# COMP6248-Reproducability-Challenge/selfsupervised-denoising

Measured on AMD Instinct MI355X. Metric: training patches/sec (64x64 gauss25 SSDN), higher is better.
Workload: dtype f16

## Files before the change

selfsupervised-denoising_amd/csrc/wgrad_body.h:

```cpp
#pragma once
#include "common.h"
#include <algorithm>
#include <cstdlib>
#include <cstring>
#include <mutex>
#include <utility>
#include <vector>
#include <type_traits>

template <int I, int N, class F>
static __device__ __forceinline__ void static_for(F&& f) {
    if constexpr (I < N) {
        f(std::integral_constant<int, I>{});
        static_for<I + 1, N>(f);
    }
}

#define WG_THREADS 256
#define WG_WAVES 4

typedef __attribute__((__vector_size__(4 * sizeof(__fp16)))) __fp16 fp16x4_t;
typedef __attribute__((address_space(3))) fp16x4_t lds_fp16x4;

static __device__ __forceinline__ half4 tr16(const char* lds_addr) {
// ... 697 lines not shown
#pragma unroll
        for (int u = 0; u < NPD; ++u) {
            const int f = tid + u * WGN_THREADS;
            const int q = f / NPD, cc = f - q * NPD;
            *reinterpret_cast<half8*>(dt + q * DSTR + cc * 16) = pd[u];
        }
#pragma unroll
        for (int u = 0; u < 2; ++u) {
            const int hp = tid + u * WGN_THREADS;
            if (hp < 324) *reinterpret_cast<half8*>(xt + hp * 16) = cvt_h8_to_bf8(px[u]);
        }
    };

    int it = 0;
    const int t0 = (int)bx;
    if (t0 < ntiles) { fetch(t0); stage(0); }
    __syncthreads();
    for (int tile = t0; tile < ntiles; tile += (int)gdx, ++it) {
        const int nxt = tile + (int)gdx;
        if (nxt < ntiles) fetch(nxt);
        const char* dt = smem + (it & 1) * (DB + XB);
        const char* xt = dt + DB;
#pragma unroll
        for (int j = 0; j < 4; ++j) {
            const int row = wave + 4 * j;
            const char* ab = dt + (row << 4) * DSTR + dlane0;
            half8 af[MT];
#pragma unroll
            for (int mt = 0; mt < MT; ++mt) af[mt] = cat8(tr16(ab + mt * 64), tr16(ab + 4 * DSTR + mt * 64));
            const char* bp = xt + row * (18 * 16) + boff;
            u16x8 bv;
#pragma unroll
            for (int q = 0; q < 8; ++q) bv[q] = *reinterpret_cast<const unsigned short*>(bp + q * 16);
            if (bmode != 0) {
#pragma unroll
                for (int q = 0; q < 8; ++q) bv[q] = bmode == 1 ? (unsigned short)0x3f80 : (unsigned short)0;
            }
            const half8 bfrag = __builtin_bit_cast(half8, bv);
#pragma unroll
            for (int mt = 0; mt < MT; ++mt)
                acc[mt] = __builtin_amdgcn_mfma_f32_32x32x16_bf16(__builtin_bit_cast(bf16x8, af[mt]), __builtin_bit_cast(bf16x8, bfrag), acc[mt], 0, 0, 0);
        }
        __syncthreads();
        if (nxt < ntiles) stage((it + 1) & 1);
        __syncthreads();
    }
    float* red = reinterpret_cast<float*>(smem);
#pragma unroll
    for (int mt = 0; mt < MT; ++mt)
#pragma unroll
        for (int r = 0; r < 16; ++r) red[((wave * MT + mt) * 16 + r) * 64 + lane] = acc[mt][r];
    __syncthreads();
    float* slab = a.slab + (long long)bx * 9 * a.Mpad * a.Kpad;
    for (int o = tid; o < MT * 16 * 64; o += WGN_THREADS) {
        const int ln = o & 63, r = (o >> 6) & 15, mt = o >> 10;
        float sum = 0.f;
#pragma unroll
        for (int w4 = 0; w4 < 4; ++w4) sum += red[((w4 * MT + mt) * 16 + r) * 64 + ln];
        const int n = ln & 31, m = mt * 32 + 8 * (r >> 2) + 4 * (ln >> 5) + (r & 3);
        if (m >= a.Mpad) continue;
        if (n < ncol) {
            const int t = n / a.kreal, c = n - t * a.kreal;
            slab[((long long)t * a.Mpad + m) * a.Kpad + c] = sum;
        } else if (n == ncol) {
            a.bslab[(long long)bx * a.Mpad + m] = sum;
        }
    }
}
static bool wgrad_thin_ok(const ssdn_wgrad_args* a) {
    static const bool off = ssdn_tuning_env("SSDN_NO_THIN_WGRAD") != nullptr;
    if (off || a->kreal < 1 || a->kreal > 3 || a->ntaps != 9 || a->csplit > 1 || a->mblocks > 1) return false;
    if ((a->H & 15) || (a->W & 15) || (a->M & 7) || a->Mpad > 96 || a->Kpad < a->kreal) return false;
    if (a->c0 > 0 ? (a->up0 || a->c1 > 0) : a->c1 <= 0) return false;
    const ssdn_view& v = a->c0 > 0 ? a->src0 : a->src1;
    if ((v.cs & 7) || (v.co & 7) || (a->dz.cs & 7) || (a->dz.co & 7)) return false;
    int mny = 0, mxy = 0, mnx = 0, mxx = 0;
    for (int t = 0; t < 9; ++t) {
        if (a->coff[t] != 0) return false;
        mny = a->dy[t] < mny ? a->dy[t] : mny; mxy = a->dy[t] > mxy ? a->dy[t] : mxy;
        mnx = a->dx[t] < mnx ? a->dx[t] : mnx; mxx = a->dx[t] > mxx ? a->dx[t] : mxx;
    }
    return mxy - mny == 2 && mxx - mnx == 2;
}
```

selfsupervised-denoising_amd/csrc/wgrad_mega.hip:

```cpp
#include "wgrad_body.h"

namespace { std::mutex g_wg_multi_mutex; }


struct WgMegaEntry {
    ssdn_wgrad_args a;
    WgAux x;
    int inst, gx, gy, pad;
};
struct WgMegaItem { int entry, bx, by, pad; };
#define WG_MEGA_INSTANCES(X) \
    X(0, 3, 7, 4, false, 192, 8, 3, 2) X(1, 3, 5, 4, false, 192, 8, 3, 2) X(2, 2, 5, 4, false, 192, 8, 3, 2) \
    X(3, 3, 4, 6, true, 832, 4, 2, 2) X(4, 3, 4, 4, false, 0, 0, 0, 0) X(5, 3, 5, 4, false, 0, 0, 0, 0) \
    X(6, 2, 5, 4, false, 0, 0, 0, 0) X(7, 1, 1, 4, false, 0, 0, 0, 0) X(8, 3, 1, 4, false, 0, 0, 0, 0) \
    X(10, 3, 5, 6, true, 0, 0, 0, 0) X(11, 2, 5, 6, true, 0, 0, 0, 0) \
    X(12, 3, 4, 6, true, 0, 0, 0, 0) X(13, 1, 1, 6, true, 0, 0, 0, 0) X(14, 3, 1, 6, true, 0, 0, 0, 0) \
    X(15, 3, 5, 2, false, 192, 8, 3, 2) X(16, 2, 5, 2, false, 192, 8, 3, 2)
typedef const __attribute__((address_space(4))) WgMegaEntry* WgMegaEntryC;
typedef const __attribute__((address_space(4))) WgMegaItem* WgMegaItemC;
__global__ __launch_bounds__(WG_THREADS) void k_wgrad_mega(const WgMegaEntry* __restrict__ ent, const WgMegaItem* __restrict__ items) {
    const unsigned long long t_start = __builtin_amdgcn_s_memrealtime();
    const WgMegaItemC it = (WgMegaItemC)(unsigned long long)(items + blockIdx.x);
    const WgMegaEntryC E4 = (WgMegaEntryC)(unsigned long long)(ent + it->entry);
    const unsigned bx = (unsigned)it->bx, by = (unsigned)it->by;
    const WgMegaEntry& E = *(const WgMegaEntry*)E4;
    const unsigned gx = (unsigned)E.gx;
    switch (E.inst) {
#define WG_X(id, mt, cpw, nl, both, ps, ks, rwx, rwd) case id: wgrad_body<mt, cpw, nl, both, ps, ks, rwx, rwd>(E.a, E.x, bx, by, gx); break;
        WG_MEGA_INSTANCES(WG_X)
#undef WG_X
        case 101: wgrad_thin_body<1>(E.a, bx, gx); break;
        case 102: wgrad_thin_body<2>(E.a, bx, gx); break;
        case 103: wgrad_thin_body<3>(E.a, bx, gx); break;
        default: break;
    }
    {
        unsigned long long* tr = E.x.trace;
        if (tr && threadIdx.x == 0) {
            tr[3 * blockIdx.x] = t_start;
            tr[3 * blockIdx.x + 1] = __builtin_amdgcn_s_memrealtime();
            tr[3 * blockIdx.x + 2] = (unsigned long long)it->entry | ((unsigned long long)bx << 16);
        }
    }
}

struct WgVariant { int thin, mt, cpw, nl, both, ps, ks, rwx, rwd; };
static WgVariant wgrad_variant(const ssdn_wgrad_args* a, const WgPrep& p) {
    WgVariant v = {};
    v.mt = p.MT; v.cpw = p.CPW;
    if (wgrad_thin_ok(a)) { v.thin = 1; return v; }
    const WgGeom& g = p.g;
    const WgItems& wi = p.wi;
    const int ksteps = (g.TN * g.TH * g.TW) >> 4;
    const bool st = !wi.both && !wi.sync && a->ltn == 0 && a->ltw >= 3 && g.ntiles > a->nslabs;
    const bool st8 = st && g.PSTR == 192 && ksteps == 8 && wi.rswx == 3 && wi.rswd == 2;
    const bool st16 = st && g.PSTR == 64 && ksteps == 16 && wi.rswx == 5 && wi.rswd == 4;
    const bool st4b = wi.both && !wi.sync && a->ltn == 0 && a->ltw >= 3 && g.ntiles > a->nslabs && g.PSTR == 832 && ksteps == 4 && wi.rswx == 2 && wi.rswd == 2;
    v.nl = wi.both ? 6 : 4; v.both = wi.both ? 1 : 0;
    if (st4b && v.mt == 3 && v.cpw == 4) { v.ps = 832; v.ks = 4; v.rwx = 2; v.rwd = 2; }
    else if (wi.both) {}
    else if (st8 && v.mt >= 2 && v.cpw >= 2) { v.ps = 192; v.ks = 8; v.rwx = 3; v.rwd = 2; if (wgrad_nl2(a, g, v.mt, v.cpw)) v.nl = 2; }
    else if (st16 && v.mt >= 2 && v.cpw <= 3) { v.ps = 64; v.ks = 16; v.rwx = 5; v.rwd = 4; }
    return v;
}
static int wgrad_mega_inst(const WgVariant& v) {
    if (v.thin) return v.mt >= 1 && v.mt <= 3 ? 100 + v.mt : -1;
#define WG_X(id, mt_, cpw_, nl_, both_, ps_, ks_, rwx_, rwd_) \
    if (v.mt == mt_ && v.cpw == cpw_ && v.nl == nl_ && (v.both != 0) == both_ && v.ps == ps_ && v.ks == ks_ && v.rwx == rwx_ && v.rwd == rwd_) return id;
    WG_MEGA_INSTANCES(WG_X)
#undef WG_X
    return -1;
}
static int wgrad_mega_prepare(const ssdn_wgrad_args* a, WgPrep* p) {
    int rc = wgrad_prepare(a, p);
    if (rc) return rc;
    if (wgrad_thin_ok(a)) {
        p->gx = a->nslabs; p->gy = 1;
        p->lds = 2 * ((size_t)256 * wg_stride(p->MT * 64) + 18 * 18 * 16);
        const size_t red = (size_t)4 * p->MT * 16 * 64 * 4;
        p->lds = p->lds > red ? p->lds : red;
    }
    return 0;
}
int wgrad_mega_ok(const ssdn_wgrad_args* a) {
    if (!a || a->mega <= 0) return 0;
    WgPrep p;
    if (wgrad_mega_prepare(a, &p)) return 0;
    return wgrad_mega_inst(wgrad_variant(a, p)) >= 0 ? 1 : 0;
}
extern "C" int ssdn_wgrad_variant(const ssdn_wgrad_args* a, int32_t* out9) {
    WgPrep p;
    int rc = wgrad_mega_prepare(a, &p);
    if (rc) return rc < -1 ? rc : -2;
    const WgVariant v = wgrad_variant(a, p);
    const int t[9] = {v.thin, v.mt, v.cpw, v.nl, v.both, v.ps, v.ks, v.rwx, v.rwd};
    for (int i = 0; i < 9; ++i) out9[i] = t[i];
    return wgrad_mega_inst(v);
}

namespace {
struct WgMegaCache {
    std::vector<char> key;
    char* dev;
    int device;
};
std::vector<WgMegaCache> g_wg_mega_cache;
}

int launch_wgrad_mega(const ssdn_wgrad_args* const* ops, int n, hipStream_t s) {
    if (n < 1 || n > WGRAD_MEGA_MAX) return ssdn_set_error("wgrad: bad mega run length %d", n);
    const int W = ops[0]->mega;
    if (W < 1 || W > 4096) return ssdn_set_error("wgrad: bad mega grid %d", W);
    std::vector<WgMegaEntry> ent((size_t)n);
    memset(ent.data(), 0, sizeof(WgMegaEntry) * (size_t)n);
    struct It { double cost; int e, bx, by; };
    std::vector<It> its;
    size_t lds = 0;
    double flops = 0, bytes = 0;
    for (int i = 0; i < n; ++i) {
        if (ops[i]->mega != W) return ssdn_set_error("wgrad: the ops of one merged launch disagree on its grid (%d vs %d)", ops[i]->mega, W);
        WgPrep p;
        int rc = wgrad_mega_prepare(ops[i], &p);
        if (rc) return rc;
        WgMegaEntry& e = ent[i];
        memcpy(&e.a, ops[i], sizeof(ssdn_wgrad_args));
        e.x = p.x;
        e.inst = wgrad_mega_inst(wgrad_variant(ops[i], p));
        if (e.inst < 0) return ssdn_set_error("wgrad: op %d of a merged run has no k_wgrad_mega instance (MT=%d CPW=%d both=%d)", i, p.MT, p.CPW, p.wi.both);
        e.gx = p.gx; e.gy = p.gy;
        lds = p.lds > lds ? p.lds : lds;
        const double px = (double)ops[i]->N * ops[i]->H * ops[i]->W;
        const int mb = ops[i]->mblocks > 1 ? ops[i]->mblocks : 1;
        const bool thin = e.inst >= 100;
        flops += thin ? 2.0 * px * ops[i]->M * ops[i]->kreal * ops[i]->ntaps : wgrad_flops(ops[i]);
        bytes += px * 2.0 * (ops[i]->M * mb + (thin ? ops[i]->kreal : ops[i]->Ktot));
        const double c = ops[i]->cost > 0.f ? (double)ops[i]->cost : 1.0;
        for (int by = 0; by < p.gy; ++by)
            for (int bx = 0; bx < p.gx; ++bx) {
                if (mb > 1 && (((bx >> 3) / mb) * 8 + (bx & 7)) >= ops[i]->nslabs) continue;
                its.push_back({c, i, bx, by});
            }
    }
    std::stable_sort(its.begin(), its.end(), [](const It& a, const It& b) { return a.cost > b.cost; });
    std::vector<WgMegaItem> items;
    for (const It& t : its) items.push_back({t.e, t.bx, t.by, 0});
    std::vector<int> starts(1, (int)items.size());
    const size_t b0 = sizeof(WgMegaEntry) * ent.size(), b1 = sizeof(WgMegaItem) * items.size(), b2 = sizeof(int) * starts.size();
    const size_t off_items = (b0 + 255) & ~(size_t)255, off_starts = (off_items + b1 + 255) & ~(size_t)255;
    std::vector<char> key(off_starts + b2, 0);
    memcpy(key.data(), ent.data(), b0);
    memcpy(key.data() + off_items, items.data(), b1);
    memcpy(key.data() + off_starts, starts.data(), b2);
    int dev = 0;
    SSDN_CHECK_HIP(hipGetDevice(&dev));
    char* dtab = nullptr;
    {
        std::lock_guard<std::mutex> lock(g_wg_multi_mutex);
        for (const WgMegaCache& c : g_wg_mega_cache)
            if (c.device == dev && c.key.size() == key.size() && !memcmp(c.key.data(), key.data(), key.size())) { dtab = c.dev; break; }
        if (!dtab) {
            if (g_wg_mega_cache.size() >= 64) {
                SSDN_CHECK_HIP(hipDeviceSynchronize());
                SSDN_CHECK_HIP(hipFree(g_wg_mega_cache.front().dev));
// ... 22 lines not shown
```

selfsupervised-denoising_amd/csrc/wgrad_mfma.hip:

```cpp
#include "wgrad_body.h"

template <int MT, int CPW, int NL, bool BOTH, int PS, int KS, int RWX, int RWD>
__global__ __launch_bounds__(WG_THREADS) void k_wgrad(ssdn_wgrad_args a, WgAux x) {
    wgrad_body<MT, CPW, NL, BOTH, PS, KS, RWX, RWD>(a, x, blockIdx.x, blockIdx.y, gridDim.x);
}

struct WgMultiEntry {
    ssdn_wgrad_args a;
    WgAux x;
    int first, gx, gy, inst;
};
#define WG_MULTI_INSTANCES(X) \
    X(0, 2, 1, 4, false) X(1, 2, 2, 4, false) X(2, 2, 3, 4, false) X(3, 2, 5, 4, false) \
    X(4, 3, 1, 4, false) X(5, 3, 2, 4, false) X(6, 3, 3, 4, false) X(7, 3, 4, 4, false) X(8, 3, 5, 4, false) \
    X(9, 3, 1, 6, true) X(10, 2, 1, 6, true) X(11, 3, 2, 6, true) X(12, 3, 4, 6, true) X(13, 2, 3, 6, true) \
    X(16, 2, 5, 6, true) X(17, 3, 5, 6, true) X(18, 3, 3, 6, true) X(19, 2, 2, 6, true)
__global__ __launch_bounds__(WG_THREADS) void k_wgrad_multi(const WgMultiEntry* __restrict__ tab, int n) {
    int e = 0;
    while (e + 1 < n && (int)blockIdx.x >= tab[e + 1].first) ++e;
    const WgMultiEntry& E = tab[e];
    const unsigned local = blockIdx.x - (unsigned)E.first;
    const unsigned gx = (unsigned)E.gx;
    const unsigned by = local / gx, bx = local - by * gx;
    switch (E.inst) {
#define WG_X(id, mt, cpw, nl, both) case id: wgrad_body<mt, cpw, nl, both, 0, 0, 0, 0>(E.a, E.x, bx, by, gx); break;
        WG_MULTI_INSTANCES(WG_X)
#undef WG_X
        default: break;
    }
}

int wgrad_lds_bytes(const ssdn_wgrad_args* a) {
    if (wgrad_validate(a)) return -1;
    WgGeom g = wg_geom(*a);
    if (wgrad_items(a, g).nl > 6) { ssdn_set_error("wgrad: the tile cannot be prefetched within its K-steps (too many rows / too wide rows)"); return -1; }
    return 2 * (g.XB + g.DB) + WG_ONES_BYTES;
}

template <int MT, int CPW, int NL, bool BOTH, int PS, int KS, int RWX, int RWD>
static int wgrad_launch(const ssdn_wgrad_args* a, const WgGeom& g, const WgAux& x, hipStream_t s) {
    size_t lds = 2 * ((size_t)g.XB + (size_t)g.DB) + WG_ONES_BYTES;
    if (lds > 160 * 1024) return ssdn_set_error("wgrad: tiling needs %zu B of LDS (> 160 KiB)", lds);
    static bool attr_set_dev[SSDN_MAX_DEVICES_ATTR] = {};
    bool& attr_set = attr_set_dev[ssdn_current_device_slot()];
    if (!attr_set) {
        SSDN_CHECK_HIP(hipFuncSetAttribute((const void*)k_wgrad<MT, CPW, NL, BOTH, PS, KS, RWX, RWD>, hipFuncAttributeMaxDynamicSharedMemorySize, 160 * 1024));
        attr_set = true;
    }
    double px = (double)a->N * a->H * a->W;
    prof_begin(SSDN_PROF_WGRAD, s);
    const int gy = a->csplit > 1 ? a->csplit : 1;
    const int gx = a->mblocks > 1 ? ((a->nslabs + 7) / 8) * 8 * a->mblocks : a->nslabs;
    hipLaunchKernelGGL((k_wgrad<MT, CPW, NL, BOTH, PS, KS, RWX, RWD>), dim3(gx, gy), dim3(WG_THREADS), lds, s, *a, x);
    prof_end(SSDN_PROF_WGRAD, s, wgrad_flops(a), px * 2.0 * (a->M * (a->mblocks > 1 ? a->mblocks : 1) + a->Ktot));
    return 0;
}

static int wgrad_multi_inst(const WgPrep& p) {
#define WG_X(id_, mt_, cpw_, nl_, both_) if (p.MT == mt_ && p.CPW == cpw_ && (p.wi.both != 0) == both_) return id_;
    WG_MULTI_INSTANCES(WG_X)
#undef WG_X
    return -1;
}
bool wgrad_mergeable(const ssdn_wgrad_args* a) {
    if (wgrad_thin_ok(a)) return false;
    static const long long small_px = [] { const char* e = ssdn_tuning_env("SSDN_WGRAD_SMALL_PX"); return e ? atoll(e) : 32768ll; }();
    if ((long long)a->N * a->H * a->W > small_px || a->mblocks > 1) return false;
    WgPrep p;
    if (wgrad_validate(a)) return false;
    p.g = wg_geom(*a);
    p.wi = wgrad_items(a, p.g);
    if (p.wi.nl > 6) return false;
    p.MT = a->Mpad / 32;
    const int CT = a->ntaps * (a->Kpad / 32) + 1;
    p.gy = a->csplit > 1 ? a->csplit : 1;
    p.CPW = (CT + WG_WAVES * p.gy - 1) / (WG_WAVES * p.gy);
    return wgrad_multi_inst(p) >= 0;
}

namespace {
struct WgMultiCache { std::vector<WgMultiEntry> host; WgMultiEntry* dev; int device; };
std::vector<WgMultiCache> g_wg_multi_cache;
std::mutex g_wg_multi_mutex;
}

int launch_wgrad_multi(const ssdn_wgrad_args* const* items, int n, hipStream_t s) {
    if (n < 1 || n > WGRAD_MULTI_MAX) return ssdn_set_error("wgrad: bad batch size %d", n);
    std::vector<WgMultiEntry> tab((size_t)n);
    memset(tab.data(), 0, sizeof(WgMultiEntry) * (size_t)n);
    size_t lds = 0;
    int blocks = 0;
    double flops = 0, bytes = 0;
    std::vector<std::pair<double, int>> order;
    std::vector<WgPrep> preps((size_t)n);
    for (int i = 0; i < n; ++i) {
        int rc = wgrad_prepare(items[i], &preps[i]);
        if (rc) return rc;
        const WgPrep& p = preps[i];
        const double tiles_per_wg = (double)p.g.ntiles / (items[i]->nslabs > 0 ? items[i]->nslabs : 1);
        const double cost = tiles_per_wg * (p.g.TN * p.g.TH * p.g.TW / 16) * (660.0 + 90.0 * p.CPW) +
                            (double)items[i]->ntaps * items[i]->Mpad * items[i]->Kpad * 4.0 / 10.0 / p.gy;
        order.push_back({-cost, i});
    }
    std::sort(order.begin(), order.end());
    for (int k = 0; k < n; ++k) {
        const int i = order[k].second;
        const WgPrep& p = preps[i];
        WgMultiEntry& e = tab[k];
        memcpy(&e.a, items[i], sizeof(ssdn_wgrad_args));
        e.x = p.x;
        e.inst = wgrad_multi_inst(p);
        if (e.inst < 0) return ssdn_set_error("wgrad: op %d of a merged run has no k_wgrad_multi instance (MT=%d CPW=%d both=%d)", i, p.MT, p.CPW, p.wi.both);
        e.first = blocks; e.gx = p.gx; e.gy = p.gy;
        blocks += p.gx * p.gy;
        lds = p.lds > lds ? p.lds : lds;
        const double px = (double)items[i]->N * items[i]->H * items[i]->W;
        flops += wgrad_flops(items[i]);
        bytes += px * 2.0 * (items[i]->M + items[i]->Ktot);
    }
    int dev = 0;
    SSDN_CHECK_HIP(hipGetDevice(&dev));
    WgMultiEntry* dtab = nullptr;
    {
        std::lock_guard<std::mutex> lock(g_wg_multi_mutex);
        for (const WgMultiCache& c : g_wg_multi_cache)
            if (c.device == dev && c.host.size() == tab.size() && !memcmp(c.host.data(), tab.data(), sizeof(WgMultiEntry) * tab.size())) { dtab = c.dev; break; }
        if (!dtab) {
            if (g_wg_multi_cache.size() >= 64) {
                SSDN_CHECK_HIP(hipDeviceSynchronize());
                SSDN_CHECK_HIP(hipFree(g_wg_multi_cache.front().dev));
                g_wg_multi_cache.erase(g_wg_multi_cache.begin());
            }
            SSDN_CHECK_HIP(hipMalloc((void**)&dtab, sizeof(WgMultiEntry) * tab.size()));
            SSDN_CHECK_HIP(hipMemcpy(dtab, tab.data(), sizeof(WgMultiEntry) * tab.size(), hipMemcpyHostToDevice));
            g_wg_multi_cache.push_back({tab, dtab, dev});
        }
    }
    static bool attr_set_dev[SSDN_MAX_DEVICES_ATTR] = {};
    bool& attr_set = attr_set_dev[ssdn_current_device_slot()];
    if (!attr_set) {
        SSDN_CHECK_HIP(hipFuncSetAttribute((const void*)k_wgrad_multi, hipFuncAttributeMaxDynamicSharedMemorySize, 160 * 1024));
        attr_set = true;
    }
    prof_begin(SSDN_PROF_WGRAD, s);
    hipLaunchKernelGGL(k_wgrad_multi, dim3(blocks), dim3(WG_THREADS), lds, s, (const WgMultiEntry*)dtab, n);
    prof_end(SSDN_PROF_WGRAD, s, flops, bytes);
    SSDN_CHECK_HIP(hipGetLastError());
    return 0;
}

template <int MT>
__global__ __launch_bounds__(WGN_THREADS) void k_wgrad_thin(ssdn_wgrad_args a) {
    wgrad_thin_body<MT>(a, blockIdx.x, gridDim.x);
}
template <int MT>
static int wgrad_thin_launch(const ssdn_wgrad_args* a, hipStream_t s) {
    const size_t lds = 2 * ((size_t)256 * wg_stride(MT * 64) + 18 * 18 * 16);
    static bool attr_set_dev[SSDN_MAX_DEVICES_ATTR] = {};
    bool& attr_set = attr_set_dev[ssdn_current_device_slot()];
    if (!attr_set) {
        SSDN_CHECK_HIP(hipFuncSetAttribute((const void*)k_wgrad_thin<MT>, hipFuncAttributeMaxDynamicSharedMemorySize, 160 * 1024));
        attr_set = true;
    }
    const double px = (double)a->N * a->H * a->W;
    prof_begin(SSDN_PROF_WGRAD, s);
    hipLaunchKernelGGL(k_wgrad_thin<MT>, dim3(a->nslabs), dim3(WGN_THREADS), lds, s, *a);
    prof_end(SSDN_PROF_WGRAD, s, 2.0 * px * a->M * a->kreal * 9, px * 2.0 * (a->M + a->kreal));
    SSDN_CHECK_HIP(hipGetLastError());
    return 0;
}
static int launch_wgrad_thin(const ssdn_wgrad_args* a, hipStream_t s) {
    switch (a->Mpad / 32) {
        case 1: return wgrad_thin_launch<1>(a, s);
        case 2: return wgrad_thin_launch<2>(a, s);
        default: return wgrad_thin_launch<3>(a, s);
    }
}

int launch_wgrad(const ssdn_wgrad_args* a, hipStream_t s) {
    WgPrep prep;
    int rc = wgrad_prepare(a, &prep);
    if (rc) return rc;
    if (wgrad_thin_ok(a)) return launch_wgrad_thin(a, s);
    const WgGeom& g = prep.g;
    const WgAux& x = prep.x;
    const WgItems& wi = prep.wi;
    const int MT = a->Mpad / 32;
    const int CT = a->ntaps * (a->Kpad / 32) + 1;
    const int gy = a->csplit > 1 ? a->csplit : 1;
    const int CPW = (CT + WG_WAVES * gy - 1) / (WG_WAVES * gy);
    const int ksteps = (g.TN * g.TH * g.TW) >> 4;
    const bool st = !wi.both && !wi.sync && a->ltn == 0 && a->ltw >= 3 && g.ntiles > a->nslabs;
    const bool st8 = st && g.PSTR == 192 && ksteps == 8 && wi.rswx == 3 && wi.rswd == 2;
    const bool st16 = st && g.PSTR == 64 && ksteps == 16 && wi.rswx == 5 && wi.rswd == 4;
    const bool st4b = wi.both && !wi.sync && a->ltn == 0 && a->ltw >= 3 && g.ntiles > a->nslabs && g.PSTR == 832 && ksteps == 4 && wi.rswx == 2 && wi.rswd == 2;
    if (st8 && wgrad_nl2(a, g, MT, CPW)) {
        rc = MT == 2 ? wgrad_launch<2, 5, 2, false, 192, 8, 3, 2>(a, g, x, s) : wgrad_launch<3, 5, 2, false, 192, 8, 3, 2>(a, g, x, s);
        if (rc) return rc;
        SSDN_CHECK_HIP(hipGetLastError());
        return 0;
    }
#define WG_S8(mt, cpw) ((mt) >= 2 && (cpw) >= 2)
#define WG_S16(mt, cpw) ((mt) >= 2 && (cpw) <= 3)
#define WG_S4B(mt, cpw) ((mt) == 3 && (cpw) == 4)
#define WG_CASE(mt, cpw) if (MT == mt && CPW == cpw) { \
        if (st4b && WG_S4B(mt, cpw)) rc = wgrad_launch<mt, cpw, 6, true, WG_S4B(mt, cpw) ? 832 : 0, WG_S4B(mt, cpw) ? 4 : 0, WG_S4B(mt, cpw) ? 2 : 0, WG_S4B(mt, cpw) ? 2 : 0>(a, g, x, s); \
        else if (wi.both) rc = wgrad_launch<mt, cpw, 6, true, 0, 0, 0, 0>(a, g, x, s); \
        else if (st8 && WG_S8(mt, cpw)) rc = wgrad_launch<mt, cpw, 4, false, WG_S8(mt, cpw) ? 192 : 0, WG_S8(mt, cpw) ? 8 : 0, WG_S8(mt, cpw) ? 3 : 0, WG_S8(mt, cpw) ? 2 : 0>(a, g, x, s); \
        else if (st16 && WG_S16(mt, cpw)) rc = wgrad_launch<mt, cpw, 4, false, WG_S16(mt, cpw) ? 64 : 0, WG_S16(mt, cpw) ? 16 : 0, WG_S16(mt, cpw) ? 5 : 0, WG_S16(mt, cpw) ? 4 : 0>(a, g, x, s); \
        else rc = wgrad_launch<mt, cpw, 4, false, 0, 0, 0, 0>(a, g, x, s); \
    } else
    WG_CASE(1, 1) WG_CASE(1, 2) WG_CASE(1, 3) WG_CASE(1, 4) WG_CASE(1, 5) WG_CASE(1, 6) WG_CASE(1, 7)
    WG_CASE(2, 1) WG_CASE(2, 2) WG_CASE(2, 3) WG_CASE(2, 4) WG_CASE(2, 5) WG_CASE(2, 6) WG_CASE(2, 7)
    WG_CASE(3, 1) WG_CASE(3, 2) WG_CASE(3, 3) WG_CASE(3, 4) WG_CASE(3, 5) WG_CASE(3, 6) WG_CASE(3, 7)
    rc = ssdn_set_error("wgrad: unsupported shape MT=%d CPW=%d", MT, CPW);
#undef WG_CASE
#undef WG_S8
#undef WG_S16
#undef WG_S4B
    if (rc) return rc;
    SSDN_CHECK_HIP(hipGetLastError());
    return 0;
}
```

selfsupervised-denoising_amd/ssdn/hip/graph.py:

```python
from __future__ import annotations

import os
from dataclasses import dataclass, field
from typing import Dict, List, Optional, Set, Tuple

LDS_LIMIT = 160 * 1024
CONV_LDS_PREFERRED = 80 * 1024
WGRAD_SMALL_PX = 32768
SMALL_WGRAD_G, SMALL_WGRAD_CUS = 2, 64
MID_WGRAD_PX, MID_WGRAD_G = 131072, 2
WGRAD_CU_FRAC = (3, 4)
WGRAD_MEGA = "split"
FUSE_UNROT_FWD = True
SIGN_BYTES_HEAD = True
X16_SLOTS = 16
POOL_ROUTE = True
SIGN_BYTES_CONV = True
SIGN_BYTES = True
MEGA_MIN_PX = 32768
SPLIT_HEAD_CUS = (1, 2)
SPLIT_AFTER = "decode_block_2.2"
SPLIT_GROUP0 = ("output_block", "decode_block_2.2")
MEGA_LANE = 0
WGRAD_LANE = 1
MAIN_LANE_WGRADS = ("encode_block_1.0", "encode_block_1.2")
SPLIT_SMALL_RUNS = True
CHAIN_POSTPONES = (2,)
MEGA_COST = {
    "static": (342.0, 38.8),
    "static2": (258.0, 40.2),
    "generic": (1350.0, 53.0),
    "head": (1208.0, 0.0),
    "head_mb": (1208.0, 0.0),
    "thin": (2211.0, 963.0),
    "sync_tile": 9000.0,
    "fixed": 30000.0,
    "slab_rate": 10.0,
}
TAPS_BLIND = [(ky - 2, kx - 1) for ky in range(3) for kx in range(3)]
TAPS_PLAIN = [(ky - 1, kx - 1) for ky in range(3) for kx in range(3)]
TAPS_1x1 = [(0, 0)]


def ceil_to(v: int, m: int) -> int:
    return (v + m - 1) // m * m


@dataclass
class TSpec:
    name: str
    kind: str
    shape: Tuple[int, ...]


@dataclass
class View:
    t: str
    co: int = 0


@dataclass
class Op:
    type: str
    a: dict = field(default_factory=dict)


@dataclass
class Layer:
    name: str
    M: int
    cin: int
    k: int
    c0: int
    c1: int
    c1_real: int
    w_off: int = 0
    b_off: int = 0

    @property
    def ntaps(self):
        return self.k * self.k

    @property
    def Ktot(self):
        return self.c0 + self.c1

    @property
    def Mpad_f(self):
        return ceil_to(self.M, 32)

    @property
    def Kd(self):
        return ceil_to(self.M, 16)


def net_layers(in_channels: int, out_channels: int, blindspot: bool) -> List[Layer]:
    c = in_channels
    cpad = 16
    nin = 384 if blindspot else 96
    L = [
        Layer("encode_block_1.0", 48, c, 3, cpad, 0, 0),
        Layer("encode_block_1.2", 48, 48, 3, 48, 0, 0),
        Layer("encode_block_2.0", 48, 48, 3, 48, 0, 0),
        Layer("encode_block_3.0", 48, 48, 3, 48, 0, 0),
        Layer("encode_block_4.0", 48, 48, 3, 48, 0, 0),
        Layer("encode_block_5.0", 48, 48, 3, 48, 0, 0),
        Layer("encode_block_6.0", 48, 48, 3, 48, 0, 0),
        Layer("decode_block_5.0", 96, 96, 3, 48, 48, 48),
        Layer("decode_block_5.2", 96, 96, 3, 96, 0, 0),
        Layer("decode_block_4.0", 96, 144, 3, 96, 48, 48),
        Layer("decode_block_4.2", 96, 96, 3, 96, 0, 0),
        Layer("decode_block_3.0", 96, 144, 3, 96, 48, 48),
        Layer("decode_block_3.2", 96, 96, 3, 96, 0, 0),
        Layer("decode_block_2.0", 96, 144, 3, 96, 48, 48),
        Layer("decode_block_2.2", 96, 96, 3, 96, 0, 0),
        Layer("decode_block_1.0", 96, 96 + c, 3, 96, cpad, c),
        Layer("decode_block_1.2", 96, 96, 3, 96, 0, 0),
# ... 470 lines not shown
            Mx = c_up + (c_skip if need_skip_grad else 0)
            dxs = self.grad("dxs_" + tag, N, h, w, Mx)
            g_up = self.grad("g_up_" + tag, N, h // 2, w // 2, c_up)
            if not dgrad(la, g_ta, 96, N, h, w, rt3, Mx, View(dxs), upsum=View(g_up), upsum_mask=View(up_src), upsum_c=c_up,
                         upsum_mask_sign=signs.get(up_src)):
                b.append(Op("upsum_bwd", dict(src=View(dxs), mask=View(up_src), dst=View(g_up), N=N, H=h // 2, W=w // 2, C=c_up)))
            return g_up, (View(dxs, c_up) if need_skip_grad else None)

        g_d2b, _ = dec_bwd("decode_block_1.0", "decode_block_1.2", d1a, d1b, g_d1b, d2b, 96, x16, X16_SLOTS, C, H, W, "d1", need_skip_grad=False)
        g_d3b, sk_p1 = dec_bwd("decode_block_2.0", "decode_block_2.2", d2a, d2b, g_d2b, d3b, 96, p1, 48, 48, H // 2, W // 2, "d2")
        g_d4b, sk_p2 = dec_bwd("decode_block_3.0", "decode_block_3.2", d3a, d3b, g_d3b, d4b, 96, p2, 48, 48, H // 4, W // 4, "d3")
        g_d5b, sk_p3 = dec_bwd("decode_block_4.0", "decode_block_4.2", d4a, d4b, g_d4b, d5b, 96, p3, 48, 48, H // 8, W // 8, "d4")
        g_e6, sk_p4 = dec_bwd("decode_block_5.0", "decode_block_5.2", d5a, d5b, g_d5b, e6, 48, p4, 48, 48, H // 16, W // 16, "d5")

        def enc_bwd(lname, g_out, src, h, w, tag, skip_add, act_prev):
            self._wgrad(L[lname], View(g_out), 48, View(src), 48, 0, None, 0, 48, N, h, w, t3)
            g_p = self.grad("g_p_" + tag, N, h, w, 48)
            dgrad(lname, g_out, 48, N, h, w, rt3, 48, View(g_p), add=skip_add)
            g_prev = self.grad("g_e_" + tag, N, 2 * h, 2 * w, 48)
            b.append(Op("pool_bwd", dict(act=View(act_prev), dpool=View(g_p), dz=View(g_prev), N=N, H=2 * h, W=2 * w, C=48, shifted=int(bs),
                                         route=routes.get(act_prev))))
            return g_prev

        g_e5 = enc_bwd("encode_block_6.0", g_e6, p5, H // 32, W // 32, "6", None, e5)
        g_e4 = enc_bwd("encode_block_5.0", g_e5, p4, H // 16, W // 16, "5", sk_p4, e4)
        g_e3 = enc_bwd("encode_block_4.0", g_e4, p3, H // 8, W // 8, "4", sk_p3, e3)
        g_e2 = enc_bwd("encode_block_3.0", g_e3, p2, H // 4, W // 4, "3", sk_p2, e2)
        g_e1 = enc_bwd("encode_block_2.0", g_e2, p1, H // 2, W // 2, "2", sk_p1, e1)
        self._wgrad(L["encode_block_1.2"], View(g_e1), 48, View(e0), 48, 0, None, 0, 48, N, H, W, t3)
        g_e0 = self.grad("g_e0", N, H, W, 48)
        dgrad("encode_block_1.2", g_e1, 48, N, H, W, rt3, 48, View(g_e0), mask=View(e0), mask_sign=signs.get(e0))
        if self.input_grad:
            dx32 = self.T("dx32", "f32", (B, C, H, W))
            b.append(Op("input_grad", dict(g_e0=View(g_e0), g_d1a=View(self.prefix + "g_d1a"), dst=dx32, B=B, C=C, H=H, W=W, R=self.R,
                                           taps=list(t3), layer_e="encode_block_1.0", layer_d="decode_block_1.0")))
        self._wgrad(L["encode_block_1.0"], View(g_e0), 48, None, 0, 0, View(x16), 16, C, N, H, W, t3)
        if self._mega_ops:
            self._plan_mega()
        self._schedule()

    def _plan_groups(self):
        mode = WGRAD_MEGA
        buckets = bucket_layers(self.layers, split_head=False)
        self._group_of, self._group_info = {}, {}
        for l in self.layers:
            for tag in ("/", "/skip"):
                g = 0
                if mode == "split":
                    g = 0 if (l.name + tag).startswith(SPLIT_GROUP0) else 1
                elif mode == "buckets":
                    g = next(k for k, b in enumerate(buckets) if l.name in b)
                self._group_of[l.name + tag] = g
                self._group_info[g] = (self.cus, MEGA_LANE, None)
        if mode == "split":
            self._group_info[0] = (max(1, (self.cus * SPLIT_HEAD_CUS[0]) // SPLIT_HEAD_CUS[1]), WGRAD_LANE, SPLIT_AFTER)

    def wgrad_group_of(self, layer_name: str, skip_half: bool = False) -> int:
        return self._group_of[layer_name + ("/skip" if skip_half else "/")]

    @staticmethod
    def is_skip_half(op) -> bool:
        return (op.type == "wgrad" and op.a.get("src0") is None and op.a["layer"].startswith("decode_block")) or \
            (op.type == "wreduce" and op.a.get("c_off", 0) > 0 and not op.a.get("tapblock"))

    def wgrad_group_info(self, g: int):
        return self._group_info[g]

    @staticmethod
    def _thin_ok(a) -> bool:
        if not (1 <= a["kreal"] <= 3) or len(a["taps"]) != 9 or a["mblocks"] > 1:
            return False
        if a["H"] % 16 or a["W"] % 16 or a["M"] % 8 or a["Mpad"] > 96 or a["Kpad"] < a["kreal"]:
            return False
        if a["c0"] > 0 and (a["up0"] or a["c1"] > 0):
            return False
        if a["c0"] == 0 and a["c1"] <= 0:
            return False
        if any(c != 0 for c in a["coff"]):
            return False
        dys = [t[0] for t in a["taps"]]
        dxs = [t[1] for t in a["taps"]]
        return max(dys) - min(dys) == 2 and max(dxs) - min(dxs) == 2

    def _mega_candidates(self, a):
        C_ = MEGA_COST
        N, H, W = a["N"], a["H"], a["W"]
        ntaps, Mpad, Kpad = len(a["taps"]), a["Mpad"], a["Kpad"]
        MT = Mpad // 32
        slab_bytes = ntaps * Mpad * Kpad * 4
        if self._thin_ok(a):
            ntiles = N * (H // 16) * (W // 16)
            fixed = C_["fixed"] + 9 * Mpad * 32 * 4 / C_["slab_rate"]
            return (4, 4, 0), ntiles, C_["thin"][0] + C_["thin"][1] * MT, fixed
        ctiles = ntaps * Kpad // 32 + 1
        cpw = -(-ctiles // 4)
        sync = False
        try:
            tile, ntiles = choose_wgrad_tile(N, H, W, a["taps"], max(Kpad, a["Ktot"]), Mpad, a["Ktot"], a["M"], 1)
        except ValueError:
            tile, ntiles = choose_wgrad_tile(N, H, W, a["taps"], max(Kpad, a["Ktot"]), Mpad, a["Ktot"], a["M"], 1 << 30)
            sync = True
        ltw, lth, ltn = tile
        ksteps = (1 << sum(tile)) // 16
        HW_ = (1 << ltw) + (max(t[1] for t in a["taps"]) - min(t[1] for t in a["taps"]))
        ix = -(-(HW_ * (a["Ktot"] // 8)) // 64)
        both = ix > 4
        static = (not both) and ltn == 0 and ltw >= 3 and ksteps == 8 and MT >= 2 and cpw >= 2 and _wg_stride(max(Kpad, a["Ktot"]) * 2) == 192
        if a["_cblocks"] and both:
            kind = "head_mb" if a["mblocks"] > 1 else "head"
        else:
            kind = "static" if static else "generic"
            if static and ix <= 2 and cpw == 5:
                kind = "static2"
        G = 2 if (kind == "generic" and MT * cpw > 16) else 1
        a["csplit"] = G if G > 1 else 0
        cpw = -(-ctiles // (4 * G))
        base, per = C_[kind]
        fixed = C_["fixed"] + slab_bytes / C_["slab_rate"] / G
        return tile, ntiles, ksteps * (base + per * MT * cpw) + (C_["sync_tile"] if sync else 0.0), fixed

    def _plan_mega(self):
        groups: Dict[int, list] = {}
        for op, reds in self._mega_ops:
            groups.setdefault(self.wgrad_group_of(op.a["layer"], self.is_skip_half(op)), []).append((op, reds))
        self.mega_makespan = {}
        for gi, members in sorted(groups.items()):
            W = self.wgrad_group_info(gi)[0]
            cand = []
            for op, reds in members:
                tile, ntiles, c_tile, fixed = self._mega_candidates(op.a)
                mb = max(1, op.a["mblocks"])
                G = max(1, op.a.get("csplit", 0))
                cand.append(dict(op=op, reds=reds, tile=tile, ntiles=ntiles, c_tile=c_tile, fixed=fixed, mb=mb * G, nmb=mb))
            def blocks_for(t):
                res = []
                for c in cand:
                    ns = -(-int(c["ntiles"] * c["c_tile"]) // max(1, int(t - c["fixed"])))
                    ns = max(1, min(c["ntiles"], ns, max(1, W // c["mb"])))
                    res.append((ns, -(-c["ntiles"] // ns) * c["c_tile"] + c["fixed"]))
                return res

            def makespan(blocks):
                import heapq
                items = sorted((cost for (ns, cost), c in zip(blocks, cand) for _ in range(ns * c["mb"])), reverse=True)
                free = [0.0] * W
                heapq.heapify(free)
                end = 0.0
                for it in items:
                    t0 = heapq.heappop(free)
                    heapq.heappush(free, t0 + it)
                    end = max(end, t0 + it)
                return end, sum(items) / W
            lower = sum(c["ntiles"] * c["c_tile"] * c["mb"] for c in cand) / float(W)
            best = None
            for k in range(120):
                t = lower * (1.0 + 0.01 * k) + max(c["fixed"] for c in cand)
                bl = blocks_for(t)
                ms = makespan(bl)
                if best is None or ms[0] < best[0][0]:
                    best = (ms, bl)
            self.mega_makespan[gi] = best[0]
            for c, (ns, cost) in zip(cand, best[1]):
                c["ns"], c["cost"] = ns, cost
            for c in cand:
                a = c["op"].a
                ns, mb = c["ns"], c["nmb"]
                a["nslabs"], (a["ltw"], a["lth"], a["ltn"]) = ns, c["tile"]
                a["mega"], a["cost"] = W, float(c["cost"])
                ntaps = len(a["taps"])
                a["slab"] = self.T("slab%d" % a["_id"], "f32", (mb * ns * ntaps * a["Mpad"] * a["Kpad"],))
                a["bslab"] = self.T("bslab%d" % a["_id"], "f32", (mb * ns * a["Mpad"],))
                for r in c["reds"]:
                    r.a["nslabs"], r.a["slab"], r.a["bslab"] = ns, a["slab"], a["bslab"]

    def _schedule(self):
        bwd = self.bwd
        side = [i for i, op in enumerate(bwd) if op.type in SIDE_OPS]
        place = (self._place_mega if self._mega_ops else self._place_layers)(side)
        order = sorted(range(len(bwd)), key=lambda i: place[i][0] if i in place else (i, -2))
# ... 46 lines not shown
```

Baseline: 21150.

## Add specialized thin-output 1x1 wgrad kernel for 96-in/16-out layers

Adds a dedicated weight-gradient kernel for 1x1 convolutions with 96 input channels and 16 output channels (likely the final output layer). It streams 256-pixel tiles through double-buffered LDS with buffer loads and uses bf16 MFMA. Three waves compute the weight slab, and a fourth multiplies by ones to produce the bias gradient. It is wired into the mega-kernel dispatch, the standalone launcher and the Python cost model, replacing the generic tiled path, which is poorly suited to such a thin M dimension. Inputs are converted from fp16 to bf16, which can slightly change precision.

```diff
diff --git a/selfsupervised-denoising_amd/csrc/wgrad_body.h b/selfsupervised-denoising_amd/csrc/wgrad_body.h
--- a/selfsupervised-denoising_amd/csrc/wgrad_body.h
+++ b/selfsupervised-denoising_amd/csrc/wgrad_body.h
@@ -803,3 +803,118 @@
     }
     return mxy - mny == 2 && mxx - mnx == 2;
 }
+
+#define WGO_XB (256 * 192)
+#define WGO_DB (256 * 32)
+#define WGO_LDS (2 * (WGO_XB + WGO_DB))
+static __device__ __forceinline__ void wgrad_thinout_body(const ssdn_wgrad_args& a, const unsigned bx, const unsigned gdx) {
+    extern __shared__ __attribute__((aligned(16))) char smem[];
+    constexpr int IMG = WGO_XB + WGO_DB;
+    const int tid = threadIdx.x, lane = tid & 63, l31 = lane & 31, kh = lane >> 5;
+    const int wave = __builtin_amdgcn_readfirstlane(tid >> 6);
+    const int i16 = lane & 15, mh = (lane >> 4) & 1;
+    const bool use0 = a.c0 > 0;
+    const h16* xp = (const h16*)(use0 ? a.src0.p : a.src1.p) + (use0 ? a.src0.co : a.src1.co);
+    const int xcs = use0 ? a.src0.cs : a.src1.cs;
+    const h16* dzp = (const h16*)a.dz.p + a.dz.co;
+    const int dcs = a.dz.cs;
+    const int P = a.N * a.H * a.W;
+    const int ntiles = (P + 255) >> 8;
+    const int ntl = (int)bx < ntiles ? (ntiles - (int)bx + (int)gdx - 1) / (int)gdx : 0;
+    const int xnum = ((P - 1) * xcs + 96) * 2, dnum = ((P - 1) * dcs + 16) * 2;
+
+    int xrel[12], drel[2];
+#pragma unroll
+    for (int u = 0; u < 12; ++u) {
+        const int f = tid + 256 * u, q = f / 12, cc = f - q * 12;
+        xrel[u] = (q * xcs + cc * 8) * 2;
+    }
+#pragma unroll
+    for (int u = 0; u < 2; ++u) {
+        const int f = tid + 256 * u;
+        drel[u] = ((f >> 1) * dcs + (f & 1) * 8) * 2;
+    }
+    auto fetch = [&](int i, half8* fx, half8* fd) __attribute__((always_inline)) {
+        const bool live = i < ntl;
+        const int p0 = ((int)bx + i * (int)gdx) << 8;
+        __amdgpu_buffer_rsrc_t rx = __builtin_amdgcn_make_buffer_rsrc((void*)xp, 0, live ? xnum : 0, SSDN_BUFFER_RSRC_FLAGS);
+        __amdgpu_buffer_rsrc_t rd = __builtin_amdgcn_make_buffer_rsrc((void*)dzp, 0, live ? dnum : 0, SSDN_BUFFER_RSRC_FLAGS);
+        const int sx = live ? p0 * xcs * 2 : 0, sd = live ? p0 * dcs * 2 : 0;
+#pragma unroll
+        for (int u = 0; u < 2; ++u) fd[u] = __builtin_bit_cast(half8, __builtin_amdgcn_raw_buffer_load_b128(rd, drel[u] + sd, 0, 0));
+#pragma unroll
+        for (int u = 0; u < 12; ++u) fx[u] = __builtin_bit_cast(half8, __builtin_amdgcn_raw_buffer_load_b128(rx, xrel[u] + sx, 0, 0));
+    };
+    auto stage = [&](int buf, const half8* fx, const half8* fd) __attribute__((always_inline)) {
+        char* xt = smem + buf * IMG + tid * 16;
+#pragma unroll
+        for (int u = 0; u < 2; ++u) *reinterpret_cast<half8*>(xt + WGO_XB + u * 4096) = fd[u];
+#pragma unroll
+        for (int u = 0; u < 12; ++u) *reinterpret_cast<half8*>(xt + u * 4096) = cvt_h8_to_bf8(fx[u]);
+    };
+
+    f32x16 acc0, acc1;
+#pragma unroll
+    for (int r = 0; r < 16; ++r) acc0[r] = acc1[r] = 0.f;
+    half8 ones;
+    {
+        u16x8 o;
+#pragma unroll
+        for (int i = 0; i < 8; ++i) o[i] = 0x3f80;
+        ones = __builtin_bit_cast(half8, o);
+    }
+    const int aoff = WGO_XB + (kh * 8 + (i16 >> 2)) * 32 + (i16 & 3) * 8;
+    const int boff = (kh * 8 + (i16 >> 2)) * 192 + (i16 & 3) * 8 + mh * 32 + (wave < 3 ? wave : 0) * 64;
+    auto compute = [&](int buf) __attribute__((always_inline)) {
+        const char* img = smem + buf * IMG;
+#pragma unroll
+        for (int ks = 0; ks < 16; ++ks) {
+            const char* ap = img + aoff + ks * (16 * 32);
+            const half8 af = mask_h8(cat8(tr16(ap), tr16(ap + 4 * 32)), mh == 0);
+            half8 bfr = ones;
+            if (wave < 3) {
+                const char* bp = img + boff + ks * (16 * 192);
+                bfr = cat8(tr16(bp), tr16(bp + 4 * 192));
+            }
+            if (ks & 1) acc1 = __builtin_amdgcn_mfma_f32_32x32x16_bf16(__builtin_bit_cast(bf16x8, af), __builtin_bit_cast(bf16x8, bfr), acc1, 0, 0, 0);
+            else acc0 = __builtin_amdgcn_mfma_f32_32x32x16_bf16(__builtin_bit_cast(bf16x8, af), __builtin_bit_cast(bf16x8, bfr), acc0, 0, 0, 0);
+        }
+    };
+
+    half8 xa[12], da[2], xb[12], db[2];
+    fetch(0, xa, da);
+    fetch(1, xb, db);
+    if (ntl > 0) stage(0, xa, da);
+    __syncthreads();
+    for (int i = 0; i < ntl; i += 2) {
+        fetch(i + 2, xa, da);
+        compute(0);
+        if (i + 1 < ntl) stage(1, xb, db);
+        __syncthreads();
+        if (i + 1 < ntl) {
+            fetch(i + 3, xb, db);
+            compute(1);
+            if (i + 2 < ntl) stage(0, xa, da);
+            __syncthreads();
+        }
+    }
+
+    float* slab = a.slab + (long long)bx * a.Mpad * a.Kpad;
+#pragma unroll
+    for (int r = 0; r < 16; ++r) {
+        const int m = 8 * (r >> 2) + 4 * kh + (r & 3);
+        const float v = acc0[r] + acc1[r];
+        if (wave < 3) slab[m * a.Kpad + wave * 32 + l31] = v;
+        else if (l31 == 0) a.bslab[(long long)bx * a.Mpad + m] = v;
+    }
+}
+static bool wgrad_thinout_ok(const ssdn_wgrad_args* a) {
+    static const bool off = ssdn_tuning_env("SSDN_NO_THINOUT_WGRAD") != nullptr;
+    if (off || a->ntaps != 1 || a->dy[0] != 0 || a->dx[0] != 0 || a->coff[0] != 0 || a->csplit > 1 || a->mblocks > 1) return false;
+    if (a->Ktot != 96 || a->Kpad != 96 || a->Mpad != 32 || a->M != 16) return false;
+    if (a->c0 > 0 ? (a->up0 || a->c1 > 0 || a->c0 != 96) : a->c1 != 96) return false;
+    const ssdn_view& v = a->c0 > 0 ? a->src0 : a->src1;
+    if ((v.cs & 7) || (v.co & 7) || (a->dz.cs & 7) || (a->dz.co & 7) || v.cs < 96 || a->dz.cs < 16) return false;
+    const long long P = (long long)a->N * a->H * a->W;
+    return P >= 1 && P * v.cs * 2 < (1ll << 30) && P * a->dz.cs * 2 < (1ll << 30);
+}
diff --git a/selfsupervised-denoising_amd/csrc/wgrad_mega.hip b/selfsupervised-denoising_amd/csrc/wgrad_mega.hip
--- a/selfsupervised-denoising_amd/csrc/wgrad_mega.hip
+++ b/selfsupervised-denoising_amd/csrc/wgrad_mega.hip
@@ -32,6 +32,7 @@
         case 101: wgrad_thin_body<1>(E.a, bx, gx); break;
         case 102: wgrad_thin_body<2>(E.a, bx, gx); break;
         case 103: wgrad_thin_body<3>(E.a, bx, gx); break;
+        case 110: wgrad_thinout_body(E.a, bx, gx); break;
         default: break;
     }
     {
@@ -49,6 +50,7 @@
     WgVariant v = {};
     v.mt = p.MT; v.cpw = p.CPW;
     if (wgrad_thin_ok(a)) { v.thin = 1; return v; }
+    if (wgrad_thinout_ok(a)) { v.thin = 2; return v; }
     const WgGeom& g = p.g;
     const WgItems& wi = p.wi;
     const int ksteps = (g.TN * g.TH * g.TW) >> 4;
@@ -64,6 +66,7 @@
     return v;
 }
 static int wgrad_mega_inst(const WgVariant& v) {
+    if (v.thin == 2) return 110;
     if (v.thin) return v.mt >= 1 && v.mt <= 3 ? 100 + v.mt : -1;
 #define WG_X(id, mt_, cpw_, nl_, both_, ps_, ks_, rwx_, rwd_) \
     if (v.mt == mt_ && v.cpw == cpw_ && v.nl == nl_ && (v.both != 0) == both_ && v.ps == ps_ && v.ks == ks_ && v.rwx == rwx_ && v.rwd == rwd_) return id;
@@ -79,6 +82,9 @@
         p->lds = 2 * ((size_t)256 * wg_stride(p->MT * 64) + 18 * 18 * 16);
         const size_t red = (size_t)4 * p->MT * 16 * 64 * 4;
         p->lds = p->lds > red ? p->lds : red;
+    } else if (wgrad_thinout_ok(a)) {
+        p->gx = a->nslabs; p->gy = 1;
+        p->lds = WGO_LDS;
     }
     return 0;
 }
diff --git a/selfsupervised-denoising_amd/csrc/wgrad_mfma.hip b/selfsupervised-denoising_amd/csrc/wgrad_mfma.hip
--- a/selfsupervised-denoising_amd/csrc/wgrad_mfma.hip
+++ b/selfsupervised-denoising_amd/csrc/wgrad_mfma.hip
@@ -63,7 +63,7 @@
     return -1;
 }
 bool wgrad_mergeable(const ssdn_wgrad_args* a) {
-    if (wgrad_thin_ok(a)) return false;
+    if (wgrad_thin_ok(a) || wgrad_thinout_ok(a)) return false;
     static const long long small_px = [] { const char* e = ssdn_tuning_env("SSDN_WGRAD_SMALL_PX"); return e ? atoll(e) : 32768ll; }();
     if ((long long)a->N * a->H * a->W > small_px || a->mblocks > 1) return false;
     WgPrep p;
@@ -177,11 +177,30 @@
     }
 }
 
+__global__ __launch_bounds__(WG_THREADS) void k_wgrad_thinout(ssdn_wgrad_args a) {
+    wgrad_thinout_body(a, blockIdx.x, gridDim.x);
+}
+static int launch_wgrad_thinout(const ssdn_wgrad_args* a, hipStream_t s) {
+    static bool attr_set_dev[SSDN_MAX_DEVICES_ATTR] = {};
+    bool& attr_set = attr_set_dev[ssdn_current_device_slot()];
+    if (!attr_set) {
+        SSDN_CHECK_HIP(hipFuncSetAttribute((const void*)k_wgrad_thinout, hipFuncAttributeMaxDynamicSharedMemorySize, 160 * 1024));
+        attr_set = true;
+    }
+    const double px = (double)a->N * a->H * a->W;
+    prof_begin(SSDN_PROF_WGRAD, s);
+    hipLaunchKernelGGL(k_wgrad_thinout, dim3(a->nslabs), dim3(WG_THREADS), WGO_LDS, s, *a);
+    prof_end(SSDN_PROF_WGRAD, s, 2.0 * px * a->M * a->Ktot, px * 2.0 * (a->M + a->Ktot));
+    SSDN_CHECK_HIP(hipGetLastError());
+    return 0;
+}
+
 int launch_wgrad(const ssdn_wgrad_args* a, hipStream_t s) {
     WgPrep prep;
     int rc = wgrad_prepare(a, &prep);
     if (rc) return rc;
     if (wgrad_thin_ok(a)) return launch_wgrad_thin(a, s);
+    if (wgrad_thinout_ok(a)) return launch_wgrad_thinout(a, s);
     const WgGeom& g = prep.g;
     const WgAux& x = prep.x;
     const WgItems& wi = prep.wi;
diff --git a/selfsupervised-denoising_amd/ssdn/hip/graph.py b/selfsupervised-denoising_amd/ssdn/hip/graph.py
--- a/selfsupervised-denoising_amd/ssdn/hip/graph.py
+++ b/selfsupervised-denoising_amd/ssdn/hip/graph.py
@@ -33,6 +33,7 @@
     "head": (1208.0, 0.0),
     "head_mb": (1208.0, 0.0),
     "thin": (2211.0, 963.0),
+    "thin_out": 5000.0,
     "sync_tile": 9000.0,
     "fixed": 30000.0,
     "slab_rate": 10.0,
@@ -669,6 +670,16 @@
         dxs = [t[1] for t in a["taps"]]
         return max(dys) - min(dys) == 2 and max(dxs) - min(dxs) == 2
 
+    @staticmethod
+    def _thinout_ok(a) -> bool:
+        if len(a["taps"]) != 1 or tuple(a["taps"][0]) != (0, 0) or a["coff"][0] != 0 or a["mblocks"] > 1 or a.get("csplit", 0) > 1:
+            return False
+        if a["Ktot"] != 96 or a["Kpad"] != 96 or a["Mpad"] != 32 or a["M"] != 16:
+            return False
+        if a["c0"] > 0 and (a["up0"] or a["c1"] > 0):
+            return False
+        return a["N"] * a["H"] * a["W"] * 96 * 2 < (1 << 30)
+
     def _mega_candidates(self, a):
         C_ = MEGA_COST
         N, H, W = a["N"], a["H"], a["W"]
@@ -682,6 +693,12 @@
         ctiles = ntaps * Kpad // 32 + 1
         cpw = -(-ctiles // 4)
         sync = False
+        if self._thinout_ok(a):
+            try:
+                tile, _ = choose_wgrad_tile(N, H, W, a["taps"], max(Kpad, a["Ktot"]), Mpad, a["Ktot"], a["M"], 1)
+            except ValueError:
+                tile, _ = choose_wgrad_tile(N, H, W, a["taps"], max(Kpad, a["Ktot"]), Mpad, a["Ktot"], a["M"], 1 << 30)
+            return tile, -(-(N * H * W) // 256), C_["thin_out"], C_["fixed"] + slab_bytes / C_["slab_rate"]
         try:
             tile, ntiles = choose_wgrad_tile(N, H, W, a["taps"], max(Kpad, a["Ktot"]), Mpad, a["Ktot"], a["M"], 1)
         except ValueError:
```

New measurement: 21170, median of 2. No clear change (+0.1%).
